# geopolars/geopolars

Measured on AMD Instinct MI355X. Metric: predicate evals/sec (10M pts x 1k polys point-in-polygon), higher is better.
Workload: dtype f64

## Files before the change

geopolars_amd/csrc/gpk_index.h:

```cpp
#pragma once

#include "gpk_common.h"

namespace gpk {

struct GridParams {
    double x0, y0, inv_w, inv_h;
    int32_t gx, gy;
};

struct IndexView {
    const double4* bbox;
    const GridParams* grid;
    const int32_t* cell_off;
    const int32_t* items;
    int32_t gx, gy;
};

struct PartInfo {
    int32_t slab_base, row0 , nrows, n_rings;
};
constexpr int PIP_SUB = 8;
constexpr int PIP_SLAB_MUL = 2;
constexpr int PIP_FINE_LOG2 = 6;
__host__ __device__ inline int slab_row0_of(int32_t packed) { return packed & 0xFFFFFF; }
__host__ __device__ inline int slab_shift_of(int32_t packed) { return packed >> 24; }
constexpr uint32_t SUB_INDIRECT = 1u << 30;
struct SubCell {
    uint32_t part_flags;
    uint32_t e0, e1, e2;
    uint32_t labels[4];
};
struct SubCell2 {
    SubCell a;
    uint32_t b_part_flags;
    uint32_t b_e0, b_e1, b_e2;
    uint32_t pad[4];
};
constexpr uint32_t SUB2_BIT = 1u << 29;
constexpr int CHAIN_MAX = 12;
constexpr uint32_t HCHAIN_COUNT_MASK = 0xFu;
constexpr int HCHAIN_BASE_SHIFT = 4;
constexpr int HCHAIN_START_SHIFT = 8;
struct HalfCell {
    uint32_t lw[2];
    uint32_t part_flags;
    uint32_t aux_base;
};
static_assert(sizeof(HalfCell) * 2 == sizeof(SubCell), "two half-cell records overlay one SubCell");
static_assert(CHAIN_MAX <= (int)HCHAIN_COUNT_MASK, "the edge count of a chain is a 4-bit field");
constexpr int PIP_ROUTE_RMAX = 512;
struct RouteWord {
    uint32_t bmask;
    uint32_t gmask;
    uint32_t rec0;
    uint32_t pad;
};
struct PipView {
    int32_t R;
    double rx0, ry0, fw, fh, inv_fw, inv_fh;
    const uint32_t* cell;
    const uint32_t* list;
    const SubCell* sub;
    const SubCell2* sub2;
    const double2* chain_xy;
    const RouteWord* route;
    const SubCell* lrec;
    const uint32_t* part_geom;
    const PartInfo* part_info;
    const float4* part_box;
    const int32_t* ring_row0;
    const int32_t* ring_slab_base;
    const int32_t* slab_off;
    const double4* slab_edges;
    const int32_t* slab_vidx;
    const double2* slab_xy;
};
constexpr uint32_t CELL_TAG_EMPTY = 0u, CELL_TAG_SINGLE = 1u, CELL_TAG_LIST = 2u, CELL_TAG_SUB = 3u;

namespace dev {
__device__ __forceinline__ int cell_of(double v, double v0, double inv, int g) {
    return (int)fmin(fmax((v - v0) * inv, 0.0), (double)(g - 1));
}
}

}

struct gpk_index {
    gpk::IndexView v;
    gpk::PipView pip;
    gpk::GridParams host_grid;
    int device;
    int64_t n_geoms, n_coords, n_rings;
    int32_t geom_type;
    void* owned[24];
    int64_t nbytes;
    int32_t pip_lean;
    uint64_t serial;
    int32_t pip_list_heavy;
};

namespace gpk {
int32_t build_pip_index(const gpk_geoarray* a, gpk_index* ix, hipStream_t s, int list_records_mode = 1);
int32_t ring_bboxes(const gpk_geoarray* a, double4* out_dev, hipStream_t s);
int32_t affine_rows_impl(const gpk_geoarray* a, const double* matrices, int32_t mat_space, double* out_xy, int32_t out_space, hipStream_t s);
}
```

geopolars_amd/csrc/gpk_join.hip:

```cpp
#include <atomic>
#include <cstring>
#include <mutex>
#include <type_traits>

#include <rocprim/rocprim.hpp>

#include <chrono>

#include "gpk_device.h"
#include "gpk_index.h"
#include "gpk_pip.h"
#include "gpk_polypoly.h"
#include "gpk_contains.h"
#include "gpk_lineal.h"
#include "gpk_scan.h"
#include "gpk_pipshared.h"

namespace gpk {

__global__ __launch_bounds__(256) void extent_partial_kernel(const double4* __restrict__ bbox, int64_t n, double4* __restrict__ part) {
    __shared__ double red[4][4];
    double mnx = INFINITY, mny = INFINITY, mxx = -INFINITY, mxy = -INFINITY;
    for (int64_t i = (int64_t)blockIdx.x * 256 + threadIdx.x; i < n; i += (int64_t)gridDim.x * 256) {
        const double4 b = bbox[i];
// ... 1865 lines not shown
    uint2* stage = stage_bytes ? (uint2*)ws.take(stage_bytes) : nullptr;
    uint32_t* counts_dev = out_counts ? (host_out ? (uint32_t*)ws.take(counts_bytes) : out_counts) : nullptr;
    uint32_t* pairs_dev = want_pairs ? (host_out ? (uint32_t*)ws.take(pairs_bytes) : out_pairs) : nullptr;


#define J_LAUNCH(...)                          \
    do {                                       \
        auto _f = [&]() -> int32_t {           \
            GPK_LAUNCH(__VA_ARGS__);           \
            return GPK_OK;                     \
        };                                     \
        int32_t _rc = _f();                    \
        if (_rc != GPK_OK) return _rc;         \
    } while (0)

    unsigned long long* stats = join_stats_buffer();
    if (fused) {
        struct {
            DevGeo polys;
            IndexView ix;
            uint64_t serial;
        } want_cold;
        memset(&want_cold, 0, sizeof want_cold);
        want_cold.polys = right->d;
        want_cold.ix = right_index->v;
        want_cold.serial = right_index->serial;
        if (!ws.tag_matches(cold, &want_cold, sizeof want_cold)) {
            J_LAUNCH("gpk_join_prep", join_prep_kernel, dim3(1), dim3(256), 0, s, stot, 0, cold, right->d, right_index->v);
            ws.set_tag(cold, &want_cold, sizeof want_cold);
        }
    } else if (chain) {
        J_LAUNCH("gpk_join_prep", join_prep_kernel, dim3(1), dim3(256), 0, s, stot, n_super + 2, cold, right->d, right_index->v);
    } else {
        const hipError_t me = hipMemsetAsync(stot, 0, sizeof(unsigned long long) * (size_t)(n_super + 2), s);
        if (me != hipSuccess) return fail(GPK_ERR_DEVICE, "spatial_join: %s", hipGetErrorString(me));
    }
    ChainHot hot;
    memset(&hot, 0, sizeof hot);
    if (chain) {
        const PipView& pv = right_index->pip;
        hot.pts_xy = left->d.xy;
        hot.pts_validity = left->d.validity;
        hot.n_points = n;
        hot.n_tiles = n_blocks;
        hot.polys_validity = right->d.validity;
        hot.R = pv.R;
        hot.logR = 0;
        while ((1 << hot.logR) < pv.R) ++hot.logR;
        hot.rx0 = pv.rx0;
        hot.ry0 = pv.ry0;
        hot.inv_fw = pv.inv_fw;
        hot.inv_fh = pv.inv_fh;
        hot.cell = pv.cell;
        hot.half = reinterpret_cast<const HalfCell*>(pv.sub);
        hot.chain_xy = pv.chain_xy;
        hot.part_geom = pv.part_geom;
        hot.route = pv.route;
        hot.counts = counts_dev;
        hot.code = code;
        hot.block_tot = btot;
        hot.super_tot = stot;
        hot.stats = stats;
        hot.cold = cold;
        hot.stage = nullptr;
        hot.pool = reinterpret_cast<uint32_t*>(stage);
        hot.n_full_tiles = left->d.validity ? 0 : (int32_t)(n / tile_points);
        hot.inv_fw_s = pv.inv_fw * (double)PIP_SUB;
        hot.inv_fh_s = pv.inv_fh * (double)PIP_SUB;
        hot.sub_max = (double)(((uint32_t)PIP_SUB << hot.logR) - 1u);
    }
    if (flow) {
        const int64_t wgs = flow_wgs;
        FusedTail tail;
        memset(&tail, 0, sizeof tail);
        tail.pairs = (uint2*)pairs_dev;
        tail.capacity = pair_capacity;
        tail.grand = grand;
        tail.grand_host = total_out;
        tail.left_base = left_row_base;
        FusedWords fw;
        int32_t frc = fused_launch_begin(s, wgs, (int)wgs, &fw);
        if (frc != GPK_OK) return frc;
        tail.slots = fw.slots;
        tail.epoch = fw.epoch;
        tail.ticket = fw.ticket;
        tail.ticket_base = fw.ticket_base;
        tail.lost = fw.lost;
        frc = launch_pip_flow(hot, tail, (int)wgs, flow_p, s);
        fused_launch_end(s, frc == GPK_OK);
        if (frc != GPK_OK) return frc;
        *counts_dev_out = counts_dev;
        *pairs_dev_out = pairs_dev;
        *grand_out = grand;
        return GPK_OK;
    }
    if (chain)
        J_LAUNCH("gpk_pip_tile", pip_tile_chain_kernel, dim3((unsigned)((n_blocks + PIP_BLOCK / 64 - 1) / (PIP_BLOCK / 64))), dim3(PIP_BLOCK), 0, s, hot);
    else if (lean)
        J_LAUNCH("gpk_pip_tile", pip_tile_lean_kernel, dim3((unsigned)n_blocks), dim3(PIP_BLOCK), 0, s, left->d, right->d, right_index->v, pvj,
                 counts_dev, code, btot, stot, stats);
    else if (right_index->pip.R > 0)
        if (right_index->pip.sub2 && one_per_lane)
            J_LAUNCH("gpk_pip_tile", (pip_tile_kernel<true, true, 1>), dim3((unsigned)n_blocks), dim3(PIP_BLOCK), 0, s, left->d, right->d,
                     right_index->v, pvj, counts_dev, code, btot, stot, multi_pool, multi_cap, multi_top, stats);
        else if (right_index->pip.sub2)
            J_LAUNCH("gpk_pip_tile", (pip_tile_kernel<true, true>), dim3((unsigned)n_blocks), dim3(PIP_BLOCK), 0, s, left->d, right->d,
// ... 150 lines not shown

int32_t gpk_index_query_envelope(const gpk_index* idx, const double* boxes4, int64_t n_boxes, int32_t mode, uint32_t* out_counts,
                                 uint32_t* out_pairs, int64_t pair_capacity, int64_t* n_pairs, int32_t space, void* stream) {
    if (!idx || !n_pairs || (n_boxes > 0 && !boxes4)) return fail(GPK_ERR_INVALID_ARGUMENT, "NULL argument");
    if (mode != GPK_QUERY_CONTAINED && mode != GPK_QUERY_INTERSECTING) return fail(GPK_ERR_INVALID_ARGUMENT, "unknown envelope query mode %d", mode);
    if (n_boxes < 0 || pair_capacity < 0 || (pair_capacity > 0 && !out_pairs)) return fail(GPK_ERR_INVALID_ARGUMENT, "bad sizes");
    if (n_boxes > (int64_t)0x7FFFFFF0ll) return fail(GPK_ERR_INVALID_ARGUMENT, "more than 2^31 query boxes");
    *n_pairs = 0;
    GPK_TRY(require_device());
    if (n_boxes == 0) return GPK_OK;
    hipStream_t s = (hipStream_t)stream;
    gpk_geoarray left, right;
    memset(&left, 0, sizeof left);
    memset(&right, 0, sizeof right);
    left.d.type = GPK_GEOM_POINT;
    left.d.n_geoms = n_boxes;
    left.device = right.device = idx->device;
    right.d.type = idx->geom_type;
    right.d.n_geoms = idx->n_geoms;
    GPK_TRY(workspace_aux(0).begin(2 * (sizeof(double4) * (size_t)n_boxes + 256)));
    double4* boxes_dev = (double4*)workspace_aux(0).take(sizeof(double4) * (size_t)n_boxes);
    const double4* src = reinterpret_cast<const double4*>(boxes4);
    if (space != GPK_MEM_DEVICE) {
        double4* up = (double4*)workspace_aux(0).take(sizeof(double4) * (size_t)n_boxes);
        GPK_HIP(hipMemcpyAsync(up, boxes4, sizeof(double4) * (size_t)n_boxes, hipMemcpyHostToDevice, s));
        src = up;
    }
    GPK_LAUNCH("gpk_query_boxes", query_boxes_kernel, dim3((unsigned)((n_boxes + 255) / 256)), dim3(256), 0, s, src, n_boxes, boxes_dev);
    return bbox_join(&left, &right, idx, 0u, out_counts, out_pairs, pair_capacity, n_pairs, space, s,
                     mode == GPK_QUERY_CONTAINED ? REFINE_ENVELOPE_CONTAINED : REFINE_ENVELOPE_INTERSECTS, boxes_dev);
}

int32_t gpk_index_free(gpk_index* idx) {
    if (!idx) return GPK_OK;
    int cur = -1;
    (void)hipGetDevice(&cur);
    if (cur != idx->device) (void)hipSetDevice(idx->device);
    (void)hipDeviceSynchronize();
    for (int i = 0; i < 24; ++i)
        if (idx->owned[i]) cached_free(idx->owned[i]);
    if (cur >= 0 && cur != idx->device) (void)hipSetDevice(cur);
    delete idx;
    return GPK_OK;
}

int32_t gpk_index_describe(const gpk_index* idx, int64_t out[8]) {
    if (!idx || !out) return fail(GPK_ERR_INVALID_ARGUMENT, "NULL argument");
    for (int i = 0; i < 8; ++i) out[i] = 0;
    out[0] = idx->pip.R;
    out[1] = idx->pip_lean;
    out[2] = idx->pip.chain_xy != nullptr;
    out[3] = idx->pip.route != nullptr;
    out[4] = idx->pip_list_heavy;
    return GPK_OK;
}

int32_t gpk_index_nbytes(const gpk_index* idx, int64_t* out_bytes) {
    if (!idx || !out_bytes) return fail(GPK_ERR_INVALID_ARGUMENT, "NULL argument");
    *out_bytes = idx->nbytes;
    return GPK_OK;
}

int32_t gpk_index_build(const gpk_geoarray* a, void* stream, gpk_index** out) {
    return gpk_index_build_ex(a, GPK_INDEX_BBOX_GRID | GPK_INDEX_PIP, nullptr, stream, out);
}

int32_t gpk_index_build_ex(const gpk_geoarray* a, int32_t parts, const double* bbox4_dev, void* stream, gpk_index** out) {
    if (!a || !out) return fail(GPK_ERR_INVALID_ARGUMENT, "NULL argument");
    *out = nullptr;
    GPK_TRY(require_device());
    hipStream_t s = (hipStream_t)stream;
    const int64_t n = a->d.n_geoms;

    gpk_index* ix = new gpk_index;
    memset(ix, 0, sizeof *ix);
    ix->device = a->device;
    ix->n_geoms = n;
    ix->geom_type = a->d.type;
    ix->n_coords = a->d.n_coords;
    ix->n_rings = a->d.n_rings;
    {
        static std::atomic<uint64_t> next_serial{1};
        ix->serial = next_serial.fetch_add(1);
    }

    int gdim = (int)ceil(2.0 * sqrt((double)(n > 0 ? n : 1)));
    if (gdim < 1) gdim = 1;
    if (gdim > 2048) gdim = 2048;
    const int64_t n_cells = (int64_t)gdim * gdim;

    auto cleanup = [&](int32_t rc) {
        gpk_index_free(ix);
        return rc;
    };
#define IX_HIP(expr)                                                                              \
    do {                                                                                          \
        hipError_t _e = (expr);                                                                   \
        if (_e != hipSuccess)                                                                     \
            return cleanup(fail(_e == hipErrorOutOfMemory ? GPK_ERR_OOM : GPK_ERR_DEVICE,         \
                                "%s failed: %s", #expr, hipGetErrorString(_e)));                  \
    } while (0)
#define IX_TRY(expr)                             \
    do {                                         \
        int32_t _rc = (expr);                    \
        if (_rc != GPK_OK) return cleanup(_rc);  \
    } while (0)
// ... 229 lines not shown
```

geopolars_amd/csrc/gpk_pipflow.hip:

```cpp
#include "gpk_pipshared.h"

namespace gpk {

constexpr int FLOW_P_MAX = 8;
constexpr int FLOW_BLOCK = 1024, FLOW_W = FLOW_BLOCK / 64;
constexpr int FLOW_ITEMS = 128;
constexpr int FLOW_PASS_AT = 40;
constexpr int FLOW_MAX_TILES = 1536;
constexpr int FLOW_ID_BITS = 22;
constexpr uint32_t FLOW_DEAD = 0xFFFFFFFFu;
constexpr uint32_t FLOW_MULTI = 0x80000000u;
constexpr uint32_t FLOW_PEND = FLOW_MULTI;
static_assert(64 * FLOW_P_MAX == 512, "an entry keeps the row within its tile in 9 bits");
static_assert(FLOW_MAX_TILES <= (1 << 14), "FlowItem::loc keeps the tile in 14 bits");

struct FlowItem {
    double px, py;
    uint32_t aux;
    uint32_t loc;
};
static_assert(sizeof(FlowItem) == 24, "list slot");

#ifdef GPK_TILE_TRACE
#define FLOW_STAMP(i)                                                                                                    \
// ... 122 lines not shown
    }
    while (wm) {
        const int j = __builtin_ctzll(wm);
        wm &= wm - 1ull;
        const double x = __shfl(qx, j, 64), y = __shfl(qy, j, 64);
        const unsigned long long cf = chain_generic_row_first_call(H_COLD(cold), x, y, lane);
        if (lane == j) flow_settle(h, s_ttot, t, slot, row, li, (uint32_t)cf, (uint32_t)(cf >> 32));
    }
    n_list -= n;
    if (n_list) {
        FlowItem keep{};
        if ((uint32_t)lane < n_list) keep = items[64 + lane];
        wave_lds_fence();
        if ((uint32_t)lane < n_list) items[lane] = keep;
    }
    wave_lds_fence();
}

typedef uint32_t u32x4 __attribute__((ext_vector_type(4)));

static __device__ __noinline__ void flow_settle_pending(const double2* pts_xy, const ChainCold* cold, uint32_t* pool, uint32_t* counts, unsigned long long* stats,
                                                        uint32_t* s_ttot, uint32_t t, uint32_t tile, uint32_t n_ent, int lane, int ts) {
    asm volatile("s_waitcnt vmcnt(0)" ::: "memory");
    uint32_t* seg = pool + ((size_t)tile << ts);
    for (uint32_t i = 0; i < n_ent; i += 64u) {
        const uint32_t e = i + (uint32_t)lane < n_ent ? __hip_atomic_load(seg + i + lane, __ATOMIC_RELAXED, __HIP_MEMORY_SCOPE_AGENT) : 0u;
        unsigned long long pm = __ballot((e & ~511u) == FLOW_PEND);
        while (pm) {
            const int j = __builtin_ctzll(pm);
            pm &= pm - 1ull;
            const uint32_t li = (uint32_t)__shfl((int)e, j, 64) & 511u, row = (tile << ts) + li, slot = i + (uint32_t)j;
            const double2 q = pts_xy[row];
            const unsigned long long cf = chain_generic_row_first_call(cold, q.x, q.y, lane);
            const uint32_t cnt = (uint32_t)cf, first = (uint32_t)(cf >> 32);
            if (lane == 0) {
                if (stats) atomicAdd(&stats[2], 1ull);
                if (cnt == 0u) {
                    seg[slot] = FLOW_DEAD;
                    if (counts) counts[row] = 0u;
                    atomicSub(&s_ttot[t], 1u);
                } else if (cnt == 1u) {
                    seg[slot] = (first << 9) | li;
                } else {
                    seg[slot] = FLOW_MULTI | (cnt << 9) | li;
                    if (counts) counts[row] = cnt;
                    atomicAdd(&s_ttot[t], cnt - 1u);
                }
            }
        }
    }
}

template <bool SIMPLE, bool FULL, int P>
__device__ __forceinline__ void flow_tile(const ChainHot& h, const uint2* s_mask, const uint32_t* s_rec0, FlowItem* items, uint32_t& n_list, uint32_t t,
                                          uint32_t tile0, int lane, uint32_t* s_tcand, uint32_t* s_ttot FLOW_PHASE_ARGS) {
    constexpr int S = PIP_SUB, FLOW_TILE = 64 * P, TS = P == 8 ? 9 : (P == 4 ? 8 : (P == 2 ? 7 : 6));
    static_assert(P == 1 || P == 2 || P == 4 || P == 8, "tile sizes");
    static_assert(S == 8, "the sub-cell arithmetic below is written for 8 x 8 sub-cells");
    asm volatile("" : "+v"(lane));
    const uint32_t tile = tile0 + t;
    const int64_t base = (int64_t)tile * FLOW_TILE;
    const int64_t n_points = FULL ? 0 : H_COLD(n_points);
    const uint32_t rem = FULL ? (uint32_t)FLOW_TILE : (uint32_t)(n_points - base < (int64_t)FLOW_TILE ? n_points - base : (int64_t)FLOW_TILE);
    double px[P], py[P];
    {
        const double2* __restrict__ tile_xy = h.pts_xy + base;
        static_for<P>([&](auto K) {
            constexpr int k = decltype(K)::value;
            double2 v = make_double2(NAN, NAN);
            if (FULL || ((uint32_t)(k * 64 + lane) < rem && dev::valid_row(H_COLD(pts_validity), base + k * 64 + lane))) v = dev::load_stream(tile_xy + (k * 64 + lane));
            px[k] = v.x;
            py[k] = v.y;
        });
    }
    GPK_SCHED_FENCE();
    FLOW_PHASE(1);
    const int logR = h.logR;
    const uint32_t sub_max = ((uint32_t)S << logR) - 1u;
    uint32_t sidx4[(P + 3) / 4], gw[P];
    u32x4 rec[P];
    static_for<(P + 3) / 4>([&](auto J) { sidx4[decltype(J)::value] = 0u; });
    uint32_t sxs[P], sys_[P], r0s[P];
    uint2 ms[P];
    static_for<P>([&](auto K) {
        constexpr int k = decltype(K)::value;
        uint32_t sx = cvt_u32_sat((px[k] - h.rx0) * h.inv_fw_s), sy = cvt_u32_sat((py[k] - h.ry0) * h.inv_fh_s);
        sx = sx < sub_max ? sx : sub_max;
        sy = sy < sub_max ? sy : sub_max;
        const uint32_t at = ((sy >> 3) << (logR - 5)) + (sx >> 8);
        ms[k] = s_mask[at];
        r0s[k] = s_rec0[at];
        sxs[k] = sx;
        sys_[k] = sy;
    });
    GPK_SCHED_FENCE();
    static_for<P>([&](auto K) {
        constexpr int k = decltype(K)::value;
        const uint32_t sx = sxs[k], sy = sys_[k], bit = (sx >> 3) & 31u;
        const bool real = !__builtin_isunordered(px[k], py[k]);
        const bool has = real && ((ms[k].x >> bit) & 1u) != 0u;
        const bool want = real && !has && ((ms[k].y >> bit) & 1u) != 0u;
        sidx4[k / 4] |= (((sy & 3u) << 3) | (sx & 7u)) << (8 * (k % 4));
        rec[k] = u32x4{0u, 0u, 0u, 0u};
        gw[k] = 0u;
        if (has) {
            const uint32_t w = r0s[k] + (uint32_t)__popc(__builtin_amdgcn_ubfe(ms[k].x, 0u, bit));
            rec[k] = *reinterpret_cast<const u32x4*>(h.half + (2u * w + ((sy >> 2) & 1u)));
        }
        if (want) gw[k] = h.cell[((sy >> 3) << logR) + (sx >> 3)];
    });
    GPK_SCHED_FENCE();
    FLOW_PHASE(2);
    uint32_t run = 0u, n_new = 0u;
    bool pend = false;
    uint32_t* const tile_counts = h.counts ? h.counts + base : nullptr;
    uint32_t* const tile_pool = h.pool + ((size_t)tile << TS);
    static_for<P>([&](auto K) {
        constexpr int k = decltype(K)::value;
        const uint32_t li = (uint32_t)(k * 64 + lane);
        const uint32_t s5 = (sidx4[k / 4] >> (8 * (k % 4))) & 31u;
        const uint32_t lw = (s5 & 16u) ? rec[k].y : rec[k].x;
        const uint32_t lab = (lw >> (2u * (s5 & 15u))) & 3u;
        uint32_t r = lab ? (rec[k].z & 0x3FFFFFFFu) : CODE_NONE;
        const uint32_t g = gw[k];
        const bool single = (g & 0xC0000001u) == 0x40000000u;
        if (single) r = (g >> 1) & 0x1FFFFFFFu;
        const bool walk = g != 0u && !single;
        if (!SIMPLE) {
            if (r != CODE_NONE) {
                const uint32_t geom = h.part_geom ? h.part_geom[r] : r;
                r = dev::valid_row(h.polys_validity, geom) ? geom : CODE_NONE;
            }
        }
        if (walk) r = 0u;
        const bool mine = FULL || li < rem;
        const bool cand = mine && r != CODE_NONE;
        bool listed = cand && (lab >= 2u || walk);
        const unsigned long long mcand = __ballot(cand);
        const uint32_t rank = run + lanes_below(mcand);
        uint32_t e = (r << 9) | li;
        unsigned long long ml = __ballot(listed);
        if (ml) {
            if (__builtin_expect(n_list + n_new + (uint32_t)__popcll(ml) > (uint32_t)FLOW_ITEMS, 0)) {
                if (listed && n_list + n_new + lanes_below(ml) >= (uint32_t)FLOW_ITEMS) {
                    listed = false;
                    e = FLOW_PEND | li;
                }
                ml = __ballot(listed);
                pend = true;
            }
            if (listed) {
                FlowItem* it = items + (n_list + n_new + lanes_below(ml));
                it->px = px[k];
                it->py = py[k];
                it->aux = walk ? 0u : rec[k].w;
                it->loc = (t << 18) | (rank << 9) | li;
            }
            n_new += (uint32_t)__popcll(ml);
        }
        if (tile_counts && mine) dev::store_stream(tile_counts + li, cand ? 1u : 0u);
        if (cand) tile_pool[rank] = e;
        run += (uint32_t)__popcll(mcand);
        GPK_SCHED_FENCE();
    });
    if (lane == 0) {
        s_tcand[t] = run;
        s_ttot[t] = run;
    }
    n_list += n_new;
    FLOW_PHASE(3);
    if (__builtin_expect(pend, 0)) flow_settle_pending(h.pts_xy, H_COLD(cold), h.pool, h.counts, H_COLD(stats), s_ttot, t, tile, run, lane, TS);
}

__device__ __forceinline__ void flow_emit_chunk(const ChainHot& h, uint32_t e, uint32_t row0, uint32_t pt0, unsigned long long* out64, uint32_t room, uint32_t& done,
                                                int lane) {
    const bool live = e != FLOW_DEAD;
    const bool multi = live && (e & FLOW_MULTI) != 0u;
    const unsigned long long mm = __ballot(multi);
    if (__builtin_expect(mm == 0ull, 1)) {
        const unsigned long long m = __ballot(live);
        const uint32_t at = done + lanes_below(m);
        if (live && at < room) __builtin_nontemporal_store(((unsigned long long)(e >> 9) << 32) | (unsigned long long)(row0 + (e & 511u)), out64 + at);
        done += (uint32_t)__popcll(m);
        return;
    }
    const uint32_t n_out = !live ? 0u : (multi ? (e >> 9) & ((1u << FLOW_ID_BITS) - 1u) : 1u);
    uint32_t incl = n_out;
#pragma unroll
    for (int o = 1; o < 64; o <<= 1) {
        const uint32_t v = __shfl_up(incl, o, 64);
        if (lane >= o) incl += v;
    }
    const uint32_t at = done + incl - n_out;
    if (live && !multi && at < room) __builtin_nontemporal_store(((unsigned long long)(e >> 9) << 32) | (unsigned long long)(row0 + (e & 511u)), out64 + at);
    unsigned long long wm = mm;
    while (wm) {
        const int j = __builtin_ctzll(wm);
        wm &= wm - 1ull;
        const uint32_t lj = (uint32_t)__shfl((int)e, j, 64) & 511u, aj = (uint32_t)__shfl((int)at, j, 64);
        const double2 q = h.pts_xy[pt0 + lj];
        chain_generic_row_call(H_COLD(cold), q.x, q.y, lane, reinterpret_cast<uint2*>(out64 + aj), aj < room ? room - aj : 0u, row0 + lj);
    }
    done += (uint32_t)__shfl((int)incl, 63, 64);
}

template <bool SIMPLE, int P>
__global__ __launch_bounds__(FLOW_BLOCK) void pip_tile_flow_kernel(ChainHot h, FusedTail tail) {
    constexpr int WORDS = PIP_ROUTE_RMAX * PIP_ROUTE_RMAX / 32, W = FLOW_W, TS = P == 8 ? 9 : (P == 4 ? 8 : (P == 2 ? 7 : 6));
    __shared__ uint2 s_mask[WORDS];
    __shared__ uint32_t s_rec0[WORDS];
    __shared__ FlowItem s_items[W][FLOW_ITEMS];
    __shared__ uint32_t s_tcand[FLOW_MAX_TILES], s_ttot[FLOW_MAX_TILES];
    __shared__ uint32_t s_next, s_next2, s_wg, s_wgtot, s_gave_up;
    __shared__ unsigned long long s_part[W];
    const int lane = threadIdx.x & 63, wave = __builtin_amdgcn_readfirstlane(threadIdx.x >> 6);
    FLOW_STAMP(0);
    unsigned long long my_ticket = 0ull;
    if (threadIdx.x == 0) my_ticket = __hip_atomic_fetch_add(T_COLD(ticket), 1ull, __ATOMIC_RELAXED, __HIP_MEMORY_SCOPE_AGENT);
    {
        const int R = H_COLD(R), words = R * R / 32;
        const uint4* __restrict__ src = reinterpret_cast<const uint4*>(H_COLD(route));
        for (int i = threadIdx.x; i < words; i += FLOW_BLOCK) {
            const uint4 rw = src[i];
            s_mask[i] = make_uint2(rw.x, rw.y);
            s_rec0[i] = rw.z;
        }
    }
    FLOW_STAMP(1);
    if (threadIdx.x == 0) {
        s_wg = (uint32_t)(my_ticket - T_COLD(ticket_base));
        s_next = 0u;
        s_next2 = 0u;
        s_gave_up = 0u;
    }
    __syncthreads();
    const uint32_t wg = __builtin_amdgcn_readfirstlane(s_wg);
    const uint32_t T0 = (uint32_t)((int64_t)wg * H_COLD(n_tiles) / (int64_t)gridDim.x), T1 = (uint32_t)((int64_t)(wg + 1u) * H_COLD(n_tiles) / (int64_t)gridDim.x);
    const uint32_t nt = T1 - T0;
    const bool want_pairs = T_COLD(pairs) != nullptr;
    FLOW_STAMP(2);
    const uint32_t nf = (int64_t)T1 <= (int64_t)H_COLD(n_full_tiles) ? nt : ((int64_t)T0 >= (int64_t)H_COLD(n_full_tiles) ? 0u : (uint32_t)(H_COLD(n_full_tiles) - (int32_t)T0));
    uint32_t n_list = 0u;
#ifdef GPK_TILE_TRACE
    int n_mine = 0;
#if GPK_TILE_TRACE == 2
    unsigned long long g_phase[6] = {0ull, 0ull, 0ull, 0ull, 0ull, 0ull}, g_last = wall_clock64();
#endif
#endif
    auto draw = [&](uint32_t* counter) -> uint32_t {
        __builtin_amdgcn_wave_barrier();
        const uint32_t d = __hip_atomic_fetch_add(counter, 1u, __ATOMIC_RELAXED, __HIP_MEMORY_SCOPE_WORKGROUP);
        return __builtin_amdgcn_readfirstlane(d) >> 6;
    };
    {
        uint32_t t = draw(&s_next);
        while (t < nf) {
            const uint32_t tn = draw(&s_next);
            FLOW_PHASE(4);
            if (n_list >= (uint32_t)FLOW_PASS_AT) flow_exact_pass<TS>(h, s_items[wave], n_list, lane, s_ttot, T0);
            FLOW_PHASE(0);
            flow_tile<SIMPLE, true, P>(h, s_mask, s_rec0, s_items[wave], n_list, t, T0, lane, s_tcand, s_ttot FLOW_PHASE_PASS);
            t = tn;
#if defined(GPK_TILE_TRACE) && GPK_TILE_TRACE != 2
            if (n_mine < 6) FLOW_STAMP(3 + n_mine);
            ++n_mine;
#endif
        }
    }
    for (;;) {
        const uint32_t t = draw(&s_next2) + nf;
        if (t >= nt) break;
        if (n_list >= (uint32_t)FLOW_PASS_AT) flow_exact_pass<TS>(h, s_items[wave], n_list, lane, s_ttot, T0);
        flow_tile<SIMPLE, false, P>(h, s_mask, s_rec0, s_items[wave], n_list, t, T0, lane, s_tcand, s_ttot FLOW_PHASE_PASS);
    }
    while (n_list) flow_exact_pass<TS>(h, s_items[wave], n_list, lane, s_ttot, T0);
#if defined(GPK_TILE_TRACE) && GPK_TILE_TRACE == 2
    FLOW_PHASE(5);
    if (h.stats && lane == 0 && wave % 5 == 0 && blockIdx.x < 900u)
        for (int i = 0; i < 6; ++i) h.stats[8 + (blockIdx.x * 4 + wave / 5) * 16 + 3 + i] = g_phase[i];
#endif
    FLOW_STAMP(9);
    __syncthreads();
    FLOW_STAMP(10);
    constexpr int EM_C = P < 4 ? P : 4, EM_T = 24 / EM_C;
    uint32_t ent[EM_T][EM_C], cand[EM_T];
    auto em_request = [&](uint32_t first) {
        static_for<EM_T>([&](auto Rr) {
            constexpr int r = decltype(Rr)::value;
            const uint32_t et = first + (uint32_t)(r * W);
            cand[r] = et < nt && want_pairs ? s_tcand[et] : 0u;
            cand[r] = __builtin_amdgcn_readfirstlane(cand[r]);
            const uint32_t* seg = h.pool + ((size_t)(T0 + et) << TS);
            static_for<EM_C>([&](auto Cc) {
                constexpr int c = decltype(Cc)::value;
                ent[r][c] = FLOW_DEAD;
                if ((uint32_t)(c * 64 + lane) < cand[r]) ent[r][c] = seg[c * 64 + lane];
            });
        });
    };
    em_request((uint32_t)wave);
    if (wave == 0) {
        uint32_t carry = 0u;
        for (uint32_t c0 = 0; c0 < nt; c0 += 64u) {
            const uint32_t v = c0 + (uint32_t)lane < nt ? s_ttot[c0 + lane] : 0u;
            uint32_t incl = v;
#pragma unroll
            for (int o = 1; o < 64; o <<= 1) {
                const uint32_t a = __shfl_up(incl, o, 64);
                if (lane >= o) incl += a;
            }
            if (c0 + (uint32_t)lane < nt) s_ttot[c0 + lane] = carry + incl - v;
            carry += (uint32_t)__shfl((int)incl, 63, 64);
        }
        if (lane == 0) s_wgtot = carry;
    }
    __syncthreads();
    const unsigned long long wg_tot = (unsigned long long)s_wgtot;
    const unsigned long long epoch = T_COLD(epoch);
    unsigned long long* const slots = T_COLD(slots);
    if (threadIdx.x == 0) __hip_atomic_store(&slots[wg], (epoch << FUSED_TOTAL_BITS) | wg_tot, __ATOMIC_RELAXED, __HIP_MEMORY_SCOPE_AGENT);
    unsigned long long acc = 0;
    bool gave_up = false;
    for (unsigned b = threadIdx.x; b < wg; b += FLOW_BLOCK) {
        unsigned long long v;
        uint32_t spins = 0;
        while (((v = __hip_atomic_load(&slots[b], __ATOMIC_RELAXED, __HIP_MEMORY_SCOPE_AGENT)) >> FUSED_TOTAL_BITS) != epoch) {
// ... 97 lines not shown
```

geopolars_amd/csrc/gpk_pipindex.hip:

```cpp
#include <cstdio>
#include <cstdlib>
#include <cstring>

#include <rocprim/rocprim.hpp>

#include <chrono>

#include "gpk_device.h"
#include "gpk_index.h"
#include "gpk_pip.h"
#include "gpk_scan.h"

namespace gpk {

struct FineGrid {
    int R;
    double rx0, ry0, fw, fh, inv_fw, inv_fh, pad_x, pad_y;
};
__device__ __forceinline__ int fcol(const FineGrid& f, double x) { return dev::cell_of(x, f.rx0, f.inv_fw, f.R); }
__device__ __forceinline__ int frow(const FineGrid& f, double y) { return dev::cell_of(y, f.ry0, f.inv_fh, f.R); }

__global__ void part_geom_kernel(DevGeo a, uint32_t* __restrict__ part_geom) {
    const int64_t g = (int64_t)blockIdx.x * blockDim.x + threadIdx.x;
    if (g >= a.n_geoms) return;
// ... 684 lines not shown
            lo = lo == 0 ? ne - 1 : lo - 1;
            ++len;
            ok = len <= CHAIN_MAX;
        }
        if (ok) {
            const double cx = g.rx0 + ((double)(S * ci) + 0.5 * S) * fw2;
            int wn = 0;
            bool on = false;
            if (pip::slab_range(pv, r0, row_c, e0, e1)) {
                for (int e = e0; e < e1; ++e) {
                    int dd = pip::slab_vertex(slab_vidx[e]) - c0 - lo;
                    if (dd < 0) dd += ne;
                    if (dd < len) continue;
                    const double4 ed = pip::slab_edge(pv, e);
                    on |= dev::ring_edge(ed.x, ed.y, ed.z, ed.w, cx, cy, wn);
                }
            }
            const int64_t start = (int64_t)c0 + (int64_t)r0 * CHAIN_MAX + lo;
            if (!on && wn >= -8 && wn <= 7 && start < ((int64_t)1 << (32 - HCHAIN_START_SHIFT)))
                word = (uint32_t)len | ((uint32_t)(wn & 15) << HCHAIN_BASE_SHIFT) | ((uint32_t)start << HCHAIN_START_SHIFT);
        }
    }
    hword[2 * item + half] = word;
}
__global__ void half_chain_commit_kernel(SubCell* __restrict__ sub, int64_t n_sub, const uint32_t* __restrict__ hword) {
    const int64_t i = (int64_t)blockIdx.x * blockDim.x + threadIdx.x;
    if (i >= n_sub) return;
    const SubCell rc = sub[i];
    HalfCell* h = reinterpret_cast<HalfCell*>(sub + i);
    h[0] = HalfCell{{rc.labels[0], rc.labels[1]}, rc.part_flags & ~SUB_INDIRECT, hword[2 * i]};
    h[1] = HalfCell{{rc.labels[2], rc.labels[3]}, rc.part_flags & ~SUB_INDIRECT, hword[2 * i + 1]};
}
__global__ void route_build_kernel(const uint32_t* __restrict__ cell, int64_t n_words, RouteWord* __restrict__ route) {
    const int64_t w = (int64_t)blockIdx.x * blockDim.x + threadIdx.x;
    if (w >= n_words) return;
    RouteWord rw{0u, 0u, 0u, 0u};
    bool have = false;
    for (int i = 0; i < 32; ++i) {
        const uint32_t cw = cell[32 * w + i];
        const uint32_t tag = cw >> 30, payload = cw & 0x3FFFFFFFu;
        if (tag == CELL_TAG_SUB && !(payload & SUB2_BIT)) {
            rw.bmask |= 1u << i;
            if (!have) {
                rw.rec0 = payload;
                have = true;
            }
        } else if (cw != 0u) {
            rw.gmask |= 1u << i;
        }
    }
    route[w] = rw;
}

__global__ void route_rank_kernel(RouteWord* __restrict__ route, int R) {
    const int row = blockIdx.x * blockDim.x + threadIdx.x;
    if (row >= R) return;
    const int per_row = R / 32;
    RouteWord* rw = route + (int64_t)row * per_row;
    uint32_t base = 0u;
    bool have = false;
    for (int j = 0; j < per_row; ++j) {
        if (rw[j].bmask && !have) {
            base = rw[j].rec0;
            have = true;
        }
        rw[j].pad = rw[j].bmask ? rw[j].rec0 - base : 0u;
    }
}

__global__ void sub_work_kernel(const uint32_t* __restrict__ cell, const int32_t* __restrict__ flag, const int32_t* __restrict__ pos,
                                int64_t n_cells, int32_t* __restrict__ work_cell, uint32_t* __restrict__ work_part) {
    const int64_t c = (int64_t)blockIdx.x * blockDim.x + threadIdx.x;
    if (c >= n_cells || !flag[c]) return;
    work_cell[pos[c]] = (int32_t)c;
    work_part[pos[c]] = (cell[c] & 0x3FFFFFFFu) >> 1;
}
__global__ void lrec_assign_kernel(const uint32_t* __restrict__ cell, uint32_t* __restrict__ list, int64_t n_cells,
                                   const int32_t* __restrict__ pos, int32_t* __restrict__ work_cell, uint32_t* __restrict__ work_part) {
    const int64_t c = (int64_t)blockIdx.x * blockDim.x + threadIdx.x;
    if (c >= n_cells) return;
    const uint32_t w = cell[c];
    if ((w >> 30) != CELL_TAG_LIST) return;
    const uint32_t off = w & 0x3FFFFFFFu, m = list[off];
    int32_t o = pos[c];
    for (uint32_t t = 0; t < m; ++t) {
        const uint32_t e = list[off + 1 + t];
        if (!(e & 1u)) continue;
        work_cell[o] = (int32_t)c;
        work_part[o] = e >> 1;
        list[off + 1 + t] = ((uint32_t)o << 1) | 1u;
        ++o;
    }
}

}

using namespace gpk;

namespace {
struct Temps {
    void* p[48] = {nullptr};
    int n = 0;
    double malloc_ms = 0.0;
    size_t malloc_bytes = 0;
    template <typename T>
    int32_t alloc(T** out, size_t count) {
        const size_t bytes = sizeof(T) * (count ? count : 1);
        void* q = gpk::workspace_aux(1).take(bytes);
        if (!q) {
            const auto t0 = std::chrono::steady_clock::now();
            hipError_t e = cached_malloc(&q, bytes);
            malloc_ms += std::chrono::duration<double, std::milli>(std::chrono::steady_clock::now() - t0).count();
            malloc_bytes += bytes;
            if (e != hipSuccess) return fail(GPK_ERR_OOM, "index build: device_malloc(%zu) failed: %s", bytes, hipGetErrorString(e));
            if (n < 48) p[n++] = q;
        }
        *out = (T*)q;
        return GPK_OK;
    }
// ... 335 lines not shown
            GPK_LAUNCH("gpk_pipidx_lrec_assign", lrec_assign_kernel, blocks_for(n_cells), dim3(256), 0, s, (const uint32_t*)cell, list, n_cells,
                       (const int32_t*)lpos, work_cell, work_part);
            GPK_LAUNCH("gpk_pipidx_lrec_head", sub_head_kernel, blocks_for(n_lrec), dim3(256), 0, s, pv, g, (const int32_t*)work_cell,
                       (const uint32_t*)work_part, (int64_t)n_lrec, lrec);
            if (n_refined == 0) {
                GPK_LAUNCH("gpk_pipidx_lrec_build", (sub_build_kernel<1, true, 1>), blocks_for((int64_t)n_lrec * PIP_SUB * PIP_SUB), dim3(256), 0, s, d, pv, g,
                           (const int32_t*)nullptr, (const int32_t*)nullptr, n_cells, (const uint32_t*)cell, (const uint32_t*)list, lrec, (SubCell2*)nullptr,
                           (const int32_t*)work_cell, (const uint32_t*)work_part, (int64_t)n_lrec);
                GPK_LAUNCH("gpk_pipidx_lrec_build", (sub_build_kernel<1, true, 2>), blocks_for((int64_t)n_lrec * PIP_SUB * PIP_SUB), dim3(256), 0, s, d, pv, g,
                           (const int32_t*)nullptr, (const int32_t*)nullptr, n_cells, (const uint32_t*)cell, (const uint32_t*)list, lrec, (SubCell2*)nullptr,
                           (const int32_t*)work_cell, (const uint32_t*)work_part, (int64_t)n_lrec);
            } else {
                GPK_LAUNCH("gpk_pipidx_lrec_build", (sub_build_kernel<1, true, 0>), blocks_for((int64_t)n_lrec * PIP_SUB * PIP_SUB), dim3(256), 0, s, d, pv, g,
                           (const int32_t*)nullptr, (const int32_t*)nullptr, n_cells, (const uint32_t*)cell, (const uint32_t*)list, lrec, (SubCell2*)nullptr,
                           (const int32_t*)work_cell, (const uint32_t*)work_part, (int64_t)n_lrec);
            }
            GPK_HIP(hipStreamSynchronize(s));
        } else {
            n_lrec = 0;
        }
    }
    stamp("list-cell records");
    pv.lrec = lrec;
    if (list_len > 0 && !lrec) {
        float4* part_box = nullptr;
        GPK_HIP(cached_malloc((void**)&part_box, sizeof(float4) * (size_t)(n_parts ? n_parts : 1)));
        keep(part_box);
        GPK_LAUNCH("gpk_pipidx_part_box", part_box_kernel, blocks_for(n_parts), dim3(256), 0, s, d, n_parts, (const double4*)ring_bbox, part_box);
        pv.part_box = part_box;
        ix->nbytes += (int64_t)(sizeof(float4) * (size_t)n_parts);
    }
    const bool boundary_cells_have_records = level2_ok && !sub_overflow && n_sub2 == 0;
    ix->pip_lean = (int64_t)list_len * 8 <= (int64_t)n_sub && n_refined == 0 && boundary_cells_have_records ? 1 : 0;
    if (getenv("GPK_DEBUG_INDEX")) fprintf(stderr, "[gpk] lean join kernel eligible: %d (list %d, refined rings: %s, one-part records %d)\n", ix->pip_lean, list_len, n_refined ? "some" : "none", n_sub);
    if (ix->pip_lean && slab_vidx && n_sub > 0 && swork_cell && d.n_coords + d.n_rings * CHAIN_MAX < ((int64_t)1 << (32 - HCHAIN_START_SHIFT))) {
        const int64_t n_ext = d.n_coords + d.n_rings * CHAIN_MAX;
        double2* cxy = nullptr;
        GPK_HIP(cached_malloc((void**)&cxy, sizeof(double2) * (size_t)n_ext));
        keep(cxy);
        uint32_t* hword;
        GPK_TRY(t.alloc(&hword, (size_t)n_sub * 2 + 2));
        pv.sub = sub;
        GPK_LAUNCH("gpk_pipidx_chain_xy", chain_xy_kernel, blocks_for(n_ext), dim3(256), 0, s, d, cxy);
        GPK_LAUNCH("gpk_pipidx_half_chain", half_chain_kernel, blocks_for((int64_t)n_sub * 2), dim3(256), 0, s, d, pv, g,
                   (const int32_t*)swork_cell, (const uint32_t*)swork_part, (int64_t)n_sub, (const int32_t*)slab_vidx, (const SubCell*)sub, hword);
        GPK_LAUNCH("gpk_pipidx_chain_commit", half_chain_commit_kernel, blocks_for(n_sub), dim3(256), 0, s, sub, (int64_t)n_sub, (const uint32_t*)hword);
        pv.chain_xy = cxy;
        ix->nbytes += (int64_t)(sizeof(double2) * (size_t)n_ext);
        if (R <= PIP_ROUTE_RMAX) {
            RouteWord* route = nullptr;
            const int64_t n_words = n_cells / 32;
            GPK_HIP(cached_malloc((void**)&route, sizeof(RouteWord) * (size_t)n_words));
            keep(route);
            GPK_LAUNCH("gpk_pipidx_route", route_build_kernel, blocks_for(n_words), dim3(256), 0, s, (const uint32_t*)cell, n_words, route);
            if (R >= 32) GPK_LAUNCH("gpk_pipidx_route_rank", route_rank_kernel, dim3((unsigned)((R + 63) / 64)), dim3(64), 0, s, route, R);
            pv.route = route;
            ix->nbytes += (int64_t)(sizeof(RouteWord) * (size_t)n_words);
        }
        GPK_HIP(hipStreamSynchronize(s));
        if (getenv("GPK_DEBUG_INDEX")) fprintf(stderr, "[gpk] half-cell chains: %d records, %lld extended coordinates%s\n", n_sub, (long long)n_ext, pv.route ? ", routing image" : "");
        stamp("local chains");
    }
    ix->nbytes += (int64_t)(sizeof(SubCell) * (size_t)n_sub + sizeof(SubCell2) * (size_t)n_sub2 + sizeof(SubCell) * (size_t)n_lrec);
    ix->pip = pv;
    ix->nbytes += (int64_t)(sizeof(uint32_t) * (size_t)n_cells + sizeof(uint32_t) * (size_t)list_len + (pv.slab_edges ? sizeof(double4) : sizeof(int32_t)) * (size_t)n_edges +
                            sizeof(int32_t) * (size_t)(n_slabs + 1) + sizeof(int32_t) * (size_t)(2 * n_rings + 1) +
                            (part_geom ? sizeof(uint32_t) * (size_t)n_parts : 0) + sizeof(PartInfo) * (size_t)n_parts);
    return GPK_OK;
}

}
```

geopolars_amd/csrc/gpk_pipshared.h:

```cpp
#pragma once

#include <type_traits>

#include "gpk_device.h"
#include "gpk_index.h"

namespace gpk {

constexpr uint32_t CODE_NONE = 0xFFFFFFFFu, CODE_MULTI = 0xFFFFFFFEu;
constexpr uint32_t CODE_POOL = 0x80000000u;

#define GPK_SCHED_FENCE() __builtin_amdgcn_sched_barrier(0)
template <int N, typename F>
__device__ __forceinline__ void static_for(F&& f) {
    if constexpr (N > 0) {
        static_for<N - 1>(f);
        f(std::integral_constant<int, N - 1>{});
    }
}

struct ChainHot {
    const double2* pts_xy;
    const uint8_t* pts_validity;
    int64_t n_points, n_tiles;
    const uint8_t* polys_validity;
    int32_t R, logR;
    double rx0, ry0, inv_fw, inv_fh;
    const uint32_t* cell;
    const HalfCell* half;
    const double2* chain_xy;
    const uint32_t* part_geom;
    const RouteWord* route;
    uint32_t* counts;
    uint32_t* code;
    unsigned long long* block_tot;
    unsigned long long* super_tot;
    unsigned long long* stats;
    const struct ChainCold* cold;
    uint2* stage;
    int32_t n_full_tiles, pad;
    double inv_fw_s, inv_fh_s, sub_max;
    uint32_t* pool;
};
struct ChainCold {
    DevGeo polys;
    IndexView ix;
    GridParams grid;
};

template <bool INLINE_EXACT>
__device__ __forceinline__ uint32_t chain_generic_row(const ChainCold* __restrict__ cold, double px, double py, int lane, uint32_t* first,
                                                      uint2* emit = nullptr, uint32_t emit_room = 0u, uint32_t l = 0u) {
    const DevGeo polys = cold->polys;
    const IndexView ix = cold->ix;
    const GridParams g = cold->grid;
    uint32_t cnt = 0;
    *first = CODE_NONE;
    if (!(px == px && py == py)) return 0u;
    const int cx = dev::cell_of(px, g.x0, g.inv_w, g.gx), cy = dev::cell_of(py, g.y0, g.inv_h, g.gy);
    const int cc = cy * g.gx + cx;
    for (int q = ix.cell_off[cc]; q < ix.cell_off[cc + 1]; ++q) {
        const int j = ix.items[q];
        const double4 bb = ix.bbox[j];
        if (!(px >= bb.x && px <= bb.z && py >= bb.y && py <= bb.w) || !dev::valid_row(polys.validity, j)) continue;
        int p0, p1;
        dev::geom_parts(polys, j, p0, p1);
        bool hit = false;
        for (int part = p0; part < p1 && !hit; ++part) {
            int r0, r1;
            dev::part_rings(polys, part, r0, r1);
            int pos = dev::POS_INSIDE;
            for (int r = r0; r < r1 && pos == dev::POS_INSIDE; ++r) {
                const int c0 = polys.ring_off[r], n = polys.ring_off[r + 1] - c0;
                int wn = 0, on = 0;
                if (n == 1) {
                    const double2 s0 = polys.xy[c0];
                    on = (px == s0.x && py == s0.y) ? 1 : 0;
                }
                for (int i = lane; i + 1 < n; i += 64) {
                    const double2 s0 = polys.xy[c0 + i], s1 = polys.xy[c0 + i + 1];
                    on |= (int)(INLINE_EXACT ? dev::ring_edge_inline(s0.x, s0.y, s1.x, s1.y, px, py, wn) : dev::ring_edge(s0.x, s0.y, s1.x, s1.y, px, py, wn));
// ... 74 lines not shown
```

geopolars_amd/spatial_index.py:

```python
from __future__ import annotations

import ctypes as C
from dataclasses import dataclass
from typing import Optional

import numpy as np

from . import _abi
from ._abi import MEM_DEVICE, MEM_HOST, PREDICATES
from .geoarrow import DeviceGeoArray
from .geoseries import GeoSeries


class SpatialIndex:

    def __init__(self, series: GeoSeries, stream: int = 0, for_points: bool = True, full: bool = False, light: bool = False):
        self.series = series
        h = C.c_void_p()
        parts = _abi.INDEX_BBOX_GRID | (_abi.INDEX_PIP if for_points else 0) | (_abi.INDEX_PIP_FULL if for_points and full else 0)
        if for_points and light and not full:
            parts |= _abi.INDEX_PIP_LIGHT
        _abi.check(_abi.lib().gpk_index_build_ex(series.device().handle, parts, None, stream, C.byref(h)))
        self._h = h

    @staticmethod
    def from_device(dev: DeviceGeoArray, stream: int = 0, for_points: bool = True, bboxes=None, full: bool = False, light: bool = False) -> "SpatialIndex":
        self = SpatialIndex.__new__(SpatialIndex)
        self.series = None
        self._dev = dev
        h = C.c_void_p()
        parts = _abi.INDEX_BBOX_GRID | (_abi.INDEX_PIP if for_points else 0) | (_abi.INDEX_PIP_FULL if for_points and full else 0)
        if for_points and light and not full:
            parts |= _abi.INDEX_PIP_LIGHT
        _abi.check(_abi.lib().gpk_index_build_ex(dev.handle, parts, bboxes.data_ptr() if bboxes is not None else None, stream, C.byref(h)))
        self._h = h
        return self

    @property
    def handle(self) -> C.c_void_p:
        return self._h

    def nbytes(self) -> int:
        n = C.c_int64(0)
        _abi.check(_abi.lib().gpk_index_nbytes(self._h, C.byref(n)))
        return int(n.value)

    def describe(self) -> dict:
        out = (C.c_int64 * 8)()
        _abi.check(_abi.lib().gpk_index_describe(self._h, out))
        return {"R": int(out[0]), "lean": bool(out[1]), "chains": bool(out[2]), "route": bool(out[3]), "list_heavy": bool(out[4])}

    def query_envelopes(self, boxes, mode: str = "contained", stream: int = 0) -> tuple[np.ndarray, np.ndarray]:
        lib = _abi.lib()
        b = np.ascontiguousarray(np.asarray(boxes, dtype=np.float64).reshape(-1, 4))
        n = len(b)
        m = {"contained": _abi.QUERY_CONTAINED, "intersecting": _abi.QUERY_INTERSECTING}[mode]
        counts = np.zeros(n, dtype=np.uint32)
        n_pairs = C.c_int64(0)
        _abi.check(lib.gpk_index_query_envelope(self._h, b.ctypes.data, n, m, counts.ctypes.data, None, 0, C.byref(n_pairs), MEM_HOST, stream))
        pairs = np.zeros((int(n_pairs.value), 2), dtype=np.uint32)
        if len(pairs):
            _abi.check(lib.gpk_index_query_envelope(self._h, b.ctypes.data, n, m, counts.ctypes.data, pairs.ctypes.data, len(pairs), C.byref(n_pairs), MEM_HOST, stream))
        return pairs, counts

    def locate_in_envelope(self, lower, upper) -> np.ndarray:
        pairs, _ = self.query_envelopes([[lower[0], lower[1], upper[0], upper[1]]], "contained")
        return pairs[:, 1].astype(np.int64)

    def locate_in_envelope_intersecting(self, lower, upper) -> np.ndarray:
        pairs, _ = self.query_envelopes([[lower[0], lower[1], upper[0], upper[1]]], "intersecting")
        return pairs[:, 1].astype(np.int64)

    def free(self) -> None:
        if self._h:
            _abi.lib().gpk_index_free(self._h)
            self._h = C.c_void_p()

    def __del__(self):
        try:
            self.free()
        except Exception:
            pass


@dataclass
class SpatialJoinArgs:

    join_type: str = "inner"
    predicate: str = "intersects"
    l_suffix: Optional[str] = "_left"
    r_suffix: Optional[str] = "_right"
    l_index: Optional[SpatialIndex] = None
    r_index: Optional[SpatialIndex] = None
    l_geom_type: int = -1
    r_geom_type: int = -1


def join_pairs(
    left: GeoSeries,
    right: GeoSeries,
    predicate: str = "intersects",
    r_index: Optional[SpatialIndex] = None,
    left_row_base: int = 0,
# ... 284 lines not shown
```

Before: 115800 billion.

## Compact interior cell labels into dense routed array indexed by gmask popcount

Replaces the full R×R cell lookup for interior (gmask) cells in the flow kernel with a compacted icell array holding only cells flagged in gmask. The in-row rank is packed into the upper bits of rec0 and a per-row base is loaded into shared memory, so the index comes from a popcount like the record lookup. This shrinks the footprint the point-in-polygon hot loop touches for interior labels, aiming to improve cache hit rates. The cost is a single-block scan kernel, a host sync at index build, and a small extra LDS array.

```diff
diff --git a/geopolars_amd/csrc/gpk_index.h b/geopolars_amd/csrc/gpk_index.h
--- a/geopolars_amd/csrc/gpk_index.h
+++ b/geopolars_amd/csrc/gpk_index.h
@@ -50,11 +50,14 @@
 static_assert(sizeof(HalfCell) * 2 == sizeof(SubCell), "two half-cell records overlay one SubCell");
 static_assert(CHAIN_MAX <= (int)HCHAIN_COUNT_MASK, "the edge count of a chain is a 4-bit field");
 constexpr int PIP_ROUTE_RMAX = 512;
+constexpr int ROUTE_REC0_BITS = 18;
+static_assert(PIP_ROUTE_RMAX * PIP_ROUTE_RMAX <= (1 << ROUTE_REC0_BITS), "a record index of a routed raster fits ROUTE_REC0_BITS");
+static_assert(PIP_ROUTE_RMAX <= (1 << (32 - ROUTE_REC0_BITS)), "an in-row rank fits above rec0");
 struct RouteWord {
     uint32_t bmask;
     uint32_t gmask;
     uint32_t rec0;
-    uint32_t pad;
+    uint32_t irank;
 };
 struct PipView {
     int32_t R;
@@ -65,6 +68,7 @@
     const SubCell2* sub2;
     const double2* chain_xy;
     const RouteWord* route;
+    const uint32_t* icell;
     const SubCell* lrec;
     const uint32_t* part_geom;
     const PartInfo* part_info;
@@ -95,6 +99,7 @@
     int32_t geom_type;
     void* owned[24];
     int64_t nbytes;
+    int64_t routed_bytes[3];
     int32_t pip_lean;
     uint64_t serial;
     int32_t pip_list_heavy;
diff --git a/geopolars_amd/csrc/gpk_join.hip b/geopolars_amd/csrc/gpk_join.hip
--- a/geopolars_amd/csrc/gpk_join.hip
+++ b/geopolars_amd/csrc/gpk_join.hip
@@ -1941,6 +1941,7 @@
         hot.inv_fw = pv.inv_fw;
         hot.inv_fh = pv.inv_fh;
         hot.cell = pv.cell;
+        hot.icell = pv.icell;
         hot.half = reinterpret_cast<const HalfCell*>(pv.sub);
         hot.chain_xy = pv.chain_xy;
         hot.part_geom = pv.part_geom;
@@ -2197,6 +2198,7 @@
     out[2] = idx->pip.chain_xy != nullptr;
     out[3] = idx->pip.route != nullptr;
     out[4] = idx->pip_list_heavy;
+    for (int i = 0; i < 3; ++i) out[5 + i] = idx->routed_bytes[i];
     return GPK_OK;
 }
 
diff --git a/geopolars_amd/csrc/gpk_pipflow.hip b/geopolars_amd/csrc/gpk_pipflow.hip
--- a/geopolars_amd/csrc/gpk_pipflow.hip
+++ b/geopolars_amd/csrc/gpk_pipflow.hip
@@ -198,7 +198,7 @@
 }
 
 template <bool SIMPLE, bool FULL, int P>
-__device__ __forceinline__ void flow_tile(const ChainHot& h, const uint2* s_mask, const uint32_t* s_rec0, FlowItem* items, uint32_t& n_list, uint32_t t,
+__device__ __forceinline__ void flow_tile(const ChainHot& h, const uint2* s_mask, const uint32_t* s_rec0, const uint32_t* s_ibase, FlowItem* items, uint32_t& n_list, uint32_t t,
                                           uint32_t tile0, int lane, uint32_t* s_tcand, uint32_t* s_ttot FLOW_PHASE_ARGS) {
     constexpr int S = PIP_SUB, FLOW_TILE = 64 * P, TS = P == 8 ? 9 : (P == 4 ? 8 : (P == 2 ? 7 : 6));
     static_assert(P == 1 || P == 2 || P == 4 || P == 8, "tile sizes");
@@ -226,7 +226,7 @@
     uint32_t sidx4[(P + 3) / 4], gw[P];
     u32x4 rec[P];
     static_for<(P + 3) / 4>([&](auto J) { sidx4[decltype(J)::value] = 0u; });
-    uint32_t sxs[P], sys_[P], r0s[P];
+    uint32_t sxs[P], sys_[P], r0s[P], ibs[P];
     uint2 ms[P];
     static_for<P>([&](auto K) {
         constexpr int k = decltype(K)::value;
@@ -236,6 +236,7 @@
         const uint32_t at = ((sy >> 3) << (logR - 5)) + (sx >> 8);
         ms[k] = s_mask[at];
         r0s[k] = s_rec0[at];
+        ibs[k] = s_ibase[sy >> 3];
         sxs[k] = sx;
         sys_[k] = sy;
     });
@@ -250,10 +251,10 @@
         rec[k] = u32x4{0u, 0u, 0u, 0u};
         gw[k] = 0u;
         if (has) {
-            const uint32_t w = r0s[k] + (uint32_t)__popc(__builtin_amdgcn_ubfe(ms[k].x, 0u, bit));
+            const uint32_t w = (r0s[k] & ((1u << ROUTE_REC0_BITS) - 1u)) + (uint32_t)__popc(__builtin_amdgcn_ubfe(ms[k].x, 0u, bit));
             rec[k] = *reinterpret_cast<const u32x4*>(h.half + (2u * w + ((sy >> 2) & 1u)));
         }
-        if (want) gw[k] = h.cell[((sy >> 3) << logR) + (sx >> 3)];
+        if (want) gw[k] = h.icell[ibs[k] + (r0s[k] >> ROUTE_REC0_BITS) + (uint32_t)__popc(__builtin_amdgcn_ubfe(ms[k].y, 0u, bit))];
     });
     GPK_SCHED_FENCE();
     FLOW_PHASE(2);
@@ -355,6 +356,7 @@
     constexpr int WORDS = PIP_ROUTE_RMAX * PIP_ROUTE_RMAX / 32, W = FLOW_W, TS = P == 8 ? 9 : (P == 4 ? 8 : (P == 2 ? 7 : 6));
     __shared__ uint2 s_mask[WORDS];
     __shared__ uint32_t s_rec0[WORDS];
+    __shared__ uint32_t s_ibase[PIP_ROUTE_RMAX];
     __shared__ FlowItem s_items[W][FLOW_ITEMS];
     __shared__ uint32_t s_tcand[FLOW_MAX_TILES], s_ttot[FLOW_MAX_TILES];
     __shared__ uint32_t s_next, s_next2, s_wg, s_wgtot, s_gave_up;
@@ -366,10 +368,12 @@
     {
         const int R = H_COLD(R), words = R * R / 32;
         const uint4* __restrict__ src = reinterpret_cast<const uint4*>(H_COLD(route));
+        const int row_shift = H_COLD(logR) - 5;
         for (int i = threadIdx.x; i < words; i += FLOW_BLOCK) {
             const uint4 rw = src[i];
             s_mask[i] = make_uint2(rw.x, rw.y);
             s_rec0[i] = rw.z;
+            if ((i & ((1 << row_shift) - 1)) == 0) s_ibase[i >> row_shift] = rw.w;
         }
     }
     FLOW_STAMP(1);
@@ -405,7 +409,7 @@
             FLOW_PHASE(4);
             if (n_list >= (uint32_t)FLOW_PASS_AT) flow_exact_pass<TS>(h, s_items[wave], n_list, lane, s_ttot, T0);
             FLOW_PHASE(0);
-            flow_tile<SIMPLE, true, P>(h, s_mask, s_rec0, s_items[wave], n_list, t, T0, lane, s_tcand, s_ttot FLOW_PHASE_PASS);
+            flow_tile<SIMPLE, true, P>(h, s_mask, s_rec0, s_ibase, s_items[wave], n_list, t, T0, lane, s_tcand, s_ttot FLOW_PHASE_PASS);
             t = tn;
 #if defined(GPK_TILE_TRACE) && GPK_TILE_TRACE != 2
             if (n_mine < 6) FLOW_STAMP(3 + n_mine);
@@ -417,7 +421,7 @@
         const uint32_t t = draw(&s_next2) + nf;
         if (t >= nt) break;
         if (n_list >= (uint32_t)FLOW_PASS_AT) flow_exact_pass<TS>(h, s_items[wave], n_list, lane, s_ttot, T0);
-        flow_tile<SIMPLE, false, P>(h, s_mask, s_rec0, s_items[wave], n_list, t, T0, lane, s_tcand, s_ttot FLOW_PHASE_PASS);
+        flow_tile<SIMPLE, false, P>(h, s_mask, s_rec0, s_ibase, s_items[wave], n_list, t, T0, lane, s_tcand, s_ttot FLOW_PHASE_PASS);
     }
     while (n_list) flow_exact_pass<TS>(h, s_items[wave], n_list, lane, s_ttot, T0);
 #if defined(GPK_TILE_TRACE) && GPK_TILE_TRACE == 2
diff --git a/geopolars_amd/csrc/gpk_pipindex.hip b/geopolars_amd/csrc/gpk_pipindex.hip
--- a/geopolars_amd/csrc/gpk_pipindex.hip
+++ b/geopolars_amd/csrc/gpk_pipindex.hip
@@ -760,19 +760,46 @@
     route[w] = rw;
 }
 
-__global__ void route_rank_kernel(RouteWord* __restrict__ route, int R) {
-    const int row = blockIdx.x * blockDim.x + threadIdx.x;
-    if (row >= R) return;
-    const int per_row = R / 32;
-    RouteWord* rw = route + (int64_t)row * per_row;
-    uint32_t base = 0u;
-    bool have = false;
-    for (int j = 0; j < per_row; ++j) {
-        if (rw[j].bmask && !have) {
-            base = rw[j].rec0;
-            have = true;
-        }
-        rw[j].pad = rw[j].bmask ? rw[j].rec0 - base : 0u;
+constexpr int ROUTE_SCAN_BLOCK = 1024;
+__global__ __launch_bounds__(ROUTE_SCAN_BLOCK) void route_irank_kernel(RouteWord* route, int n_words, int per_row, int32_t* __restrict__ total) {
+    __shared__ uint32_t s_wave[ROUTE_SCAN_BLOCK / 64];
+    const int per = (n_words + ROUTE_SCAN_BLOCK - 1) / ROUTE_SCAN_BLOCK;
+    const int w0 = (int)threadIdx.x * per, w1 = w0 + per < n_words ? w0 + per : n_words;
+    uint32_t mine = 0u;
+    for (int w = w0; w < w1; ++w) mine += (uint32_t)__popc(route[w].gmask);
+    const int lane = threadIdx.x & 63, wave = threadIdx.x >> 6;
+    uint32_t incl = mine;
+#pragma unroll
+    for (int o = 1; o < 64; o <<= 1) {
+        const uint32_t v = __shfl_up(incl, o, 64);
+        if (lane >= o) incl += v;
+    }
+    if (lane == 63) s_wave[wave] = incl;
+    __syncthreads();
+    uint32_t before = incl - mine;
+    for (int i = 0; i < wave; ++i) before += s_wave[i];
+    for (int w = w0; w < w1; ++w) {
+        route[w].irank = before;
+        before += (uint32_t)__popc(route[w].gmask);
+    }
+    if (threadIdx.x == ROUTE_SCAN_BLOCK - 1) *total = (int32_t)before;
+    __syncthreads();
+    for (int w = w0; w < w1; ++w) {
+        const int first = w / per_row * per_row;
+        if (w == first) continue;
+        const uint32_t base = route[first].irank;
+        route[w].rec0 |= (route[w].irank - base) << ROUTE_REC0_BITS;
+        route[w].irank = base;
+    }
+}
+__global__ void route_icell_kernel(const uint32_t* __restrict__ cell, const RouteWord* __restrict__ route, int64_t n_words, uint32_t* __restrict__ icell) {
+    const int64_t w = (int64_t)blockIdx.x * blockDim.x + threadIdx.x;
+    if (w >= n_words) return;
+    uint32_t m = route[w].gmask, at = route[w].irank + (route[w].rec0 >> ROUTE_REC0_BITS);
+    while (m) {
+        const int i = __builtin_ctz(m);
+        m &= m - 1u;
+        icell[at++] = cell[32 * w + i];
     }
 }
 
@@ -1214,10 +1241,23 @@
             const int64_t n_words = n_cells / 32;
             GPK_HIP(cached_malloc((void**)&route, sizeof(RouteWord) * (size_t)n_words));
             keep(route);
+            int32_t* n_icell_dev;
+            GPK_TRY(t.alloc(&n_icell_dev, 64));
             GPK_LAUNCH("gpk_pipidx_route", route_build_kernel, blocks_for(n_words), dim3(256), 0, s, (const uint32_t*)cell, n_words, route);
-            if (R >= 32) GPK_LAUNCH("gpk_pipidx_route_rank", route_rank_kernel, dim3((unsigned)((R + 63) / 64)), dim3(64), 0, s, route, R);
+            GPK_LAUNCH("gpk_pipidx_route_irank", route_irank_kernel, dim3(1), dim3(ROUTE_SCAN_BLOCK), 0, s, route, (int)n_words, R >= 32 ? R / 32 : 1, n_icell_dev);
+            int32_t n_icell = 0;
+            GPK_HIP(d2h_small(&n_icell, n_icell_dev, sizeof n_icell, s));
+            GPK_HIP(sync_small(s));
+            uint32_t* icell = nullptr;
+            GPK_HIP(cached_malloc((void**)&icell, sizeof(uint32_t) * (size_t)(n_icell ? n_icell : 1)));
+            keep(icell);
+            GPK_LAUNCH("gpk_pipidx_route_icell", route_icell_kernel, blocks_for(n_words), dim3(256), 0, s, (const uint32_t*)cell, (const RouteWord*)route, n_words, icell);
             pv.route = route;
-            ix->nbytes += (int64_t)(sizeof(RouteWord) * (size_t)n_words);
+            pv.icell = icell;
+            ix->nbytes += (int64_t)(sizeof(RouteWord) * (size_t)n_words + sizeof(uint32_t) * (size_t)n_icell);
+            ix->routed_bytes[0] = (int64_t)(sizeof(HalfCell) * 2 * (size_t)n_sub);
+            ix->routed_bytes[1] = (int64_t)(sizeof(uint32_t) * (size_t)n_icell);
+            ix->routed_bytes[2] = (int64_t)(sizeof(double2) * (size_t)n_ext);
         }
         GPK_HIP(hipStreamSynchronize(s));
         if (getenv("GPK_DEBUG_INDEX")) fprintf(stderr, "[gpk] half-cell chains: %d records, %lld extended coordinates%s\n", n_sub, (long long)n_ext, pv.route ? ", routing image" : "");
diff --git a/geopolars_amd/csrc/gpk_pipshared.h b/geopolars_amd/csrc/gpk_pipshared.h
--- a/geopolars_amd/csrc/gpk_pipshared.h
+++ b/geopolars_amd/csrc/gpk_pipshared.h
@@ -27,6 +27,7 @@
     int32_t R, logR;
     double rx0, ry0, inv_fw, inv_fh;
     const uint32_t* cell;
+    const uint32_t* icell;
     const HalfCell* half;
     const double2* chain_xy;
     const uint32_t* part_geom;
diff --git a/geopolars_amd/spatial_index.py b/geopolars_amd/spatial_index.py
--- a/geopolars_amd/spatial_index.py
+++ b/geopolars_amd/spatial_index.py
@@ -48,7 +48,8 @@
     def describe(self) -> dict:
         out = (C.c_int64 * 8)()
         _abi.check(_abi.lib().gpk_index_describe(self._h, out))
-        return {"R": int(out[0]), "lean": bool(out[1]), "chains": bool(out[2]), "route": bool(out[3]), "list_heavy": bool(out[4])}
+        return {"R": int(out[0]), "lean": bool(out[1]), "chains": bool(out[2]), "route": bool(out[3]), "list_heavy": bool(out[4]),
+                "routed_record_bytes": int(out[5]), "routed_interior_bytes": int(out[6]), "routed_chain_bytes": int(out[7])}
 
     def query_envelopes(self, boxes, mode: str = "contained", stream: int = 0) -> tuple[np.ndarray, np.ndarray]:
         lib = _abi.lib()
```

After: 116700 billion, median of 6. Within noise of the previous version (+0.7%).
